# jameshball/kidney-diffusion

Hardware: AMD Instinct MI355X
Metric: denoising-steps/sec (64->256 SR UNet, bs16) (higher is better)
Workload: dtype f32

## Files before the change

kidney-diffusion_amd/csrc/kernels_small.hip:

```cpp
#include "common.h"

namespace kd {

typedef float f32x16 __attribute__((ext_vector_type(16)));
typedef float f32x4 __attribute__((ext_vector_type(4)));

__device__ __forceinline__ float act_s(float v, int act) {
  if (act == ACT_SILU) return v / (1.0f + expf(-v));
  if (act == ACT_GELU) return 0.5f * v * (1.0f + erff(v * 0.70710678118654752440f));
  if (act == ACT_SIGMOID) return 1.0f / (1.0f + expf(-v));
  return v;
}
__device__ __forceinline__ float wave_sum(float v) {
#pragma unroll
  for (int off = 32; off > 0; off >>= 1) v += __shfl_xor(v, off, 64);
  return v;
}

constexpr int SKM_UNROLL = 8;

template <int KW>
__global__ __launch_bounds__(64 * KW) void linear_skinny_mfma_kernel(const float* __restrict__ x, int ldx,
                                                                    const float* __restrict__ w,
                                                                    const float* __restrict__ bias,
                                                                    float* __restrict__ y, int ldy, int M, int K, int N,
                                                                    int in_act, int act) {
  __shared__ float part[KW > 1 ? (KW - 1) * 16 * 64 : 1];
  const int lane = threadIdx.x & 63, i = lane & 31, h = lane >> 5;
  const int kw = threadIdx.x >> 6;
  const int n0 = blockIdx.x * 32, m0 = blockIdx.y * 32;
  const int n = min(n0 + i, N - 1);
  const int m = m0 + i;
  const bool m_ok = m < M;
  const float* wp = w + (int64_t)n * K + 4 * h;
  const float* xp = x + (int64_t)(m_ok ? m : 0) * ldx + 4 * h;
  f32x16 acc;
#pragma unroll
  for (int r = 0; r < 16; ++r) acc[r] = 0.f;
  const f32x4 z = {0.f, 0.f, 0.f, 0.f};
  const int kper = KW > 1 ? ((K + KW * 8 * SKM_UNROLL - 1) / (KW * 8 * SKM_UNROLL)) * (8 * SKM_UNROLL) : K;
  const int k_lo = kw * kper, k_hi = min(K, k_lo + kper);
  for (int k0 = k_lo; k0 < k_hi; k0 += 8 * SKM_UNROLL) {
    f32x4 a[SKM_UNROLL], b[SKM_UNROLL];
#pragma unroll
    for (int u = 0; u < SKM_UNROLL; ++u) {
      int k = k0 + 8 * u + 4 * h;
      bool ok = k < k_hi;
      a[u] = ok ? *(const f32x4*)(wp + k0 + 8 * u) : z;
      b[u] = (ok && m_ok) ? *(const f32x4*)(xp + k0 + 8 * u) : z;
    }
#pragma unroll
    for (int u = 0; u < SKM_UNROLL; ++u) {
      if (in_act != ACT_NONE) {
#pragma unroll
        for (int e = 0; e < 4; ++e) b[u][e] = act_s(b[u][e], in_act);
      }
#pragma unroll
      for (int s = 0; s < 4; ++s) acc = __builtin_amdgcn_mfma_f32_32x32x2f32(a[u][s], b[u][s], acc, 0, 0, 0);
    }
  }
  if (KW > 1) {
    if (kw > 0) {
#pragma unroll
      for (int r = 0; r < 16; ++r) part[((kw - 1) * 16 + r) * 64 + lane] = acc[r];
    }
    __syncthreads();
    if (kw > 0) return;
#pragma unroll
    for (int q = 0; q < KW - 1; ++q)
#pragma unroll
      for (int r = 0; r < 16; ++r) acc[r] += part[(q * 16 + r) * 64 + lane];
  }
  if (!m_ok) return;
  float* yr = y + (int64_t)m * ldy;
  const bool vec = (ldy & 3) == 0 && (((uintptr_t)y) & 15) == 0;
#pragma unroll
  for (int g = 0; g < 4; ++g) {
    const int nb = n0 + 8 * g + 4 * h;
    float v[4];
#pragma unroll
    for (int e = 0; e < 4; ++e) {
      int nn = nb + e;
      v[e] = act_s(acc[4 * g + e] + ((bias && nn < N) ? bias[nn] : 0.f), act);
    }
    if (vec && nb + 3 < N) {
      f32x4 o = {v[0], v[1], v[2], v[3]};
      *(f32x4*)(yr + nb) = o;
    } else {
#pragma unroll
      for (int e = 0; e < 4; ++e)
        if (nb + e < N) yr[nb + e] = v[e];
    }
  }
}

int launch_linear_skinny(const float* x, int ldx, const float* w, const float* bias, float* y, int ldy, int M,
                         int K, int N, int in_act, int act, hipStream_t s) {
  KD_REQUIRE(M > 0 && N > 0 && K > 0, "skinny linear: empty");
  const bool mfma_ok = (K & 3) == 0 && (ldx & 3) == 0 && (((uintptr_t)x) & 15) == 0 && (((uintptr_t)w) & 15) == 0;
  if (!mfma_ok) return launch_linear_skinny_valu(x, ldx, w, bias, y, ldy, M, K, N, in_act, act, s);
  if (M == 1 && K <= 16384) return launch_linear_gemv(x, w, bias, y, K, N, in_act, act, s);
  dim3 grid((N + 31) / 32, (M + 31) / 32);
  if (K >= 512)
    hipLaunchKernelGGL(linear_skinny_mfma_kernel<4>, grid, dim3(256), 0, s, x, ldx, w, bias, y, ldy, M, K, N, in_act, act);
  else
    hipLaunchKernelGGL(linear_skinny_mfma_kernel<1>, grid, dim3(64), 0, s, x, ldx, w, bias, y, ldy, M, K, N, in_act, act);
  KD_HIP_CHECK(hipGetLastError());
  return 0;
}

constexpr int GCA_ROWS = 256;
static inline int gca_rows(int HW, int B) {
  int r = GCA_ROWS;
  while ((HW + r - 1) / r > 1024) r *= 2;
  while (r > 32 && (int64_t)((HW + r - 1) / r) * B < 1024 && (HW + r / 2 - 1) / (r / 2) <= 1024) r /= 2;
  return r;
}
constexpr int GCA_MAXT = 8;
constexpr int GCA_U = 4;

template <int T, int RPW>
__global__ __launch_bounds__(256) void gca_partial_kernel(const float* __restrict__ x, const float* __restrict__ wk,
                                                          const float* __restrict__ bk, float* __restrict__ part,
                                                          int HW, int C, int rows) {
  extern __shared__ float sm[];
  const int b = blockIdx.y, chunk = blockIdx.x, nchunks = gridDim.x;
  const int lane = threadIdx.x & 63, wave = threadIdx.x >> 6;
  constexpr int LPR = 64 / RPW;
  const int sub = RPW == 2 ? (lane >> 5) : 0;
  const int li = RPW == 2 ? (lane & 31) : lane;
  const int C4 = C >> 2;
  const int p0 = chunk * rows, p1 = min(HW, p0 + rows);
  f32x4 wv[T], acc[T];
  const f32x4 z = {0.f, 0.f, 0.f, 0.f};
#pragma unroll
  for (int t = 0; t < T; ++t) {
    int c4 = li + LPR * t;
    wv[t] = c4 < C4 ? *(const f32x4*)(wk + c4 * 4) : z;
    acc[t] = z;
  }
  const float bias = bk[0];
  float mrun = -INFINITY, lrun = 0.f;
  const int stride = 4 * RPW;
  for (int pb = p0 + wave * RPW + sub; pb < p1; pb += stride * GCA_U) {
    f32x4 xv[GCA_U][T];
#pragma unroll
    for (int u = 0; u < GCA_U; ++u) {
      const int p = pb + u * stride;
      const float* xr = x + ((int64_t)b * HW + (p < p1 ? p : p0)) * C;
#pragma unroll
      for (int t = 0; t < T; ++t) {
        int c4 = li + LPR * t;
        xv[u][t] = c4 < C4 ? *(const f32x4*)(xr + c4 * 4) : z;
      }
    }
#pragma unroll
    for (int u = 0; u < GCA_U; ++u) {
      float d = 0.f;
#pragma unroll
      for (int t = 0; t < T; ++t)
        d += (xv[u][t][0] * wv[t][0] + xv[u][t][1] * wv[t][1]) + (xv[u][t][2] * wv[t][2] + xv[u][t][3] * wv[t][3]);
#pragma unroll
      for (int off = LPR / 2; off > 0; off >>= 1) d += __shfl_xor(d, off, 64);
      if (pb + u * stride < p1) {
        const float logit = d + bias;
        const float mnew = fmaxf(mrun, logit);
        const float corr = expf(mrun - mnew), pw = expf(logit - mnew);
        lrun = lrun * corr + pw;
#pragma unroll
        for (int t = 0; t < T; ++t) acc[t] = acc[t] * corr + xv[u][t] * pw;
        mrun = mnew;
      }
    }
  }
  if (RPW == 2) {
    const float mo = __shfl_xor(mrun, 32, 64), lo = __shfl_xor(lrun, 32, 64);
    const float mn = fmaxf(mrun, mo);
    const float e1 = mrun == -INFINITY ? 0.f : expf(mrun - mn), e2 = mo == -INFINITY ? 0.f : expf(mo - mn);
#pragma unroll
    for (int t = 0; t < T; ++t) {
      f32x4 ao;
#pragma unroll
      for (int e = 0; e < 4; ++e) ao[e] = __shfl_xor(acc[t][e], 32, 64);
      acc[t] = acc[t] * e1 + ao * e2;
    }
    lrun = lrun * e1 + lo * e2;
    mrun = mn;
  }
  float* sacc = sm;
  float* sml = sm + 4 * C;
  if (lane == 0) {
    sml[wave * 2] = mrun;
    sml[wave * 2 + 1] = lrun;
  }
  if (sub == 0) {
#pragma unroll
    for (int t = 0; t < T; ++t) {
      int c4 = li + LPR * t;
      if (c4 < C4) *(f32x4*)(sacc + wave * C + c4 * 4) = acc[t];
    }
  }
  __syncthreads();
  float mb = fmaxf(fmaxf(sml[0], sml[2]), fmaxf(sml[4], sml[6]));
  float sc[4], lb = 0.f;
#pragma unroll
  for (int wv_ = 0; wv_ < 4; ++wv_) {
    sc[wv_] = sml[wv_ * 2] == -INFINITY ? 0.f : expf(sml[wv_ * 2] - mb);
    lb += sml[wv_ * 2 + 1] * sc[wv_];
  }
  float* out = part + ((int64_t)b * nchunks + chunk) * (C + 2);
  for (int c = threadIdx.x; c < C; c += 256)
    out[2 + c] = (sacc[c] * sc[0] + sacc[C + c] * sc[1]) + (sacc[2 * C + c] * sc[2] + sacc[3 * C + c] * sc[3]);
  if (threadIdx.x == 0) {
    out[0] = mb;
    out[1] = lb;
  }
}

__global__ __launch_bounds__(256) void gca_combine_kernel(const float* __restrict__ part, float* __restrict__ pooled,
                                                          int nchunks, int C) {
  __shared__ float se[1024];
  __shared__ float red[8];
  __shared__ float sacc[16][16];
  const int b = blockIdx.x, lane = threadIdx.x & 63, wave = threadIdx.x >> 6;
  const int cl = threadIdx.x & 15, sub = threadIdx.x >> 4;
  const int c = blockIdx.y * 16 + cl;
  const float* pb = part + (int64_t)b * nchunks * (C + 2);
  float m = -INFINITY;
  for (int i = threadIdx.x; i < nchunks; i += 256) m = fmaxf(m, pb[(int64_t)i * (C + 2)]);
#pragma unroll
  for (int off = 32; off > 0; off >>= 1) m = fmaxf(m, __shfl_xor(m, off, 64));
  if (lane == 0) red[wave] = m;
  __syncthreads();
  const float mg = fmaxf(fmaxf(red[0], red[1]), fmaxf(red[2], red[3]));
  float l = 0.f;
  for (int i = threadIdx.x; i < nchunks; i += 256) {
    float e = expf(pb[(int64_t)i * (C + 2)] - mg);
    se[i] = e;
    l += pb[(int64_t)i * (C + 2) + 1] * e;
  }
  l = wave_sum(l);
  if (lane == 0) red[4 + wave] = l;
  __syncthreads();
  const float inv = 1.0f / ((red[4] + red[5]) + (red[6] + red[7]));
  float s = 0.f;
  if (c < C)
    for (int i = sub; i < nchunks; i += 16) s += pb[(int64_t)i * (C + 2) + 2 + c] * se[i];
  sacc[sub][cl] = s;
  __syncthreads();
  if (sub == 0 && c < C) {
    float t = 0.f;
#pragma unroll
    for (int k = 0; k < 16; ++k) t += sacc[k][cl];
    pooled[(int64_t)b * C + c] = t * inv;
  }
}

constexpr int GCAG_MAXC = 512;
__global__ __launch_bounds__(256) void gca_gate_kernel(const float* __restrict__ part, int nchunks, int C,
                                                       const float* __restrict__ w0, const float* __restrict__ b0, int hid,
                                                       const float* __restrict__ w2, const float* __restrict__ b2,
                                                       float* __restrict__ gate) {
  __shared__ float se[1024];
  __shared__ float red[8];
  __shared__ __attribute__((aligned(16))) float pooled[GCAG_MAXC];
  __shared__ __attribute__((aligned(16))) float hidden[GCAG_MAXC / 2];
  const int b = blockIdx.x, lane = threadIdx.x & 63, wave = threadIdx.x >> 6;
  const float* pb = part + (int64_t)b * nchunks * (C + 2);
  float m = -INFINITY;
  for (int i = threadIdx.x; i < nchunks; i += 256) m = fmaxf(m, pb[(int64_t)i * (C + 2)]);
#pragma unroll
  for (int off = 32; off > 0; off >>= 1) m = fmaxf(m, __shfl_xor(m, off, 64));
  if (lane == 0) red[wave] = m;
  __syncthreads();
  const float mg = fmaxf(fmaxf(red[0], red[1]), fmaxf(red[2], red[3]));
  float l = 0.f;
  for (int i = threadIdx.x; i < nchunks; i += 256) {
    const float e = expf(pb[(int64_t)i * (C + 2)] - mg);
    se[i] = e;
    l += pb[(int64_t)i * (C + 2) + 1] * e;
  }
  l = wave_sum(l);
  if (lane == 0) red[4 + wave] = l;
  __syncthreads();
  const float inv = 1.0f / ((red[4] + red[5]) + (red[6] + red[7]));
  for (int c = threadIdx.x; c < C; c += 256) {
    float s0 = 0.f, s1 = 0.f, s2 = 0.f, s3 = 0.f;
    int i = 0;
    for (; i + 3 < nchunks; i += 4) {
      s0 = fmaf(pb[(int64_t)i * (C + 2) + 2 + c], se[i], s0);
      s1 = fmaf(pb[(int64_t)(i + 1) * (C + 2) + 2 + c], se[i + 1], s1);
      s2 = fmaf(pb[(int64_t)(i + 2) * (C + 2) + 2 + c], se[i + 2], s2);
      s3 = fmaf(pb[(int64_t)(i + 3) * (C + 2) + 2 + c], se[i + 3], s3);
    }
    for (; i < nchunks; ++i) s0 = fmaf(pb[(int64_t)i * (C + 2) + 2 + c], se[i], s0);
    pooled[c] = ((s0 + s1) + (s2 + s3)) * inv;
  }
  __syncthreads();
  typedef float f32x4g __attribute__((ext_vector_type(4)));
  for (int h = threadIdx.x; h < hid; h += 256) {
    const f32x4g* wr = (const f32x4g*)(w0 + (int64_t)h * C);
    float a0 = 0.f, a1 = 0.f, a2 = 0.f, a3 = 0.f;
    for (int c4 = 0; c4 < C / 4; ++c4) {
      const f32x4g wv = wr[c4], pv = *(const f32x4g*)(pooled + 4 * c4);
      a0 = fmaf(wv[0], pv[0], a0);
      a1 = fmaf(wv[1], pv[1], a1);
      a2 = fmaf(wv[2], pv[2], a2);
      a3 = fmaf(wv[3], pv[3], a3);
    }
    const float v = ((a0 + a1) + (a2 + a3)) + b0[h];
    hidden[h] = v / (1.0f + expf(-v));
  }
  __syncthreads();
  for (int n = threadIdx.x; n < C; n += 256) {
    const float* wr = w2 + (int64_t)n * hid;
    float a0 = 0.f, a1 = 0.f;
    int h = 0;
    if ((hid & 3) == 0) {
      float a2 = 0.f, a3 = 0.f;
      for (; h < hid; h += 4) {
        const f32x4g wv = *(const f32x4g*)(wr + h), hv = *(const f32x4g*)(hidden + h);
        a0 = fmaf(wv[0], hv[0], a0);
        a1 = fmaf(wv[1], hv[1], a1);
        a2 = fmaf(wv[2], hv[2], a2);
        a3 = fmaf(wv[3], hv[3], a3);
      }
      a0 += a2;
      a1 += a3;
    } else {
      for (; h < hid; ++h) a0 = fmaf(wr[h], hidden[h], a0);
    }
    const float v = (a0 + a1) + b2[n];
    gate[(int64_t)b * C + n] = 1.0f / (1.0f + expf(-v));
  }
}

bool gca_gate_fused_ok(int C, int hid) {
  return C % 4 == 0 && C <= GCAG_MAXC && hid <= GCAG_MAXC / 2 && hid > 0;
}

static int launch_gca_partial(const float* x, const float* wk, const float* bk, float* scratch, int B, int HW, int C, int rows,
                              int chunks, hipStream_t s) {
  size_t smem = (size_t)(4 * C + 8) * sizeof(float);
  const int C4 = C / 4;
  dim3 grid(chunks, B), blk(256);
  if (C4 == 32) hipLaunchKernelGGL((gca_partial_kernel<1, 2>), grid, blk, smem, s, x, wk, bk, scratch, HW, C, rows);
  else if (C4 <= 64) hipLaunchKernelGGL((gca_partial_kernel<1, 1>), grid, blk, smem, s, x, wk, bk, scratch, HW, C, rows);
  else if (C4 <= 128) hipLaunchKernelGGL((gca_partial_kernel<2, 1>), grid, blk, smem, s, x, wk, bk, scratch, HW, C, rows);
  else if (C4 <= 256) hipLaunchKernelGGL((gca_partial_kernel<4, 1>), grid, blk, smem, s, x, wk, bk, scratch, HW, C, rows);
  else hipLaunchKernelGGL((gca_partial_kernel<8, 1>), grid, blk, smem, s, x, wk, bk, scratch, HW, C, rows);
  KD_HIP_CHECK(hipGetLastError());
  return 0;
}

int launch_gca_gate(const float* x, const float* wk, const float* bk, float* scratch, const float* w0, const float* b0, int hid,
                    const float* w2, const float* b2, float* gate, int B, int HW, int C, hipStream_t s) {
  KD_REQUIRE(gca_gate_fused_ok(C, hid), "fused GlobalContext gate needs C % 4 == 0, C <= 512, hidden <= 256");
  KD_REQUIRE((((uintptr_t)w0 | (uintptr_t)w2) & 15) == 0, "fused GlobalContext gate: 16-byte aligned weights");
  const int rows = gca_rows(HW, B), chunks = (HW + rows - 1) / rows;
  if (launch_gca_partial(x, wk, bk, scratch, B, HW, C, rows, chunks, s)) return 1;
  hipLaunchKernelGGL(gca_gate_kernel, dim3(B), dim3(256), 0, s, scratch, chunks, C, w0, b0, hid, w2, b2, gate);
  KD_HIP_CHECK(hipGetLastError());
  return 0;
}

size_t gca_scratch_floats(int B, int HW, int C) {
  int rows = gca_rows(HW, B), chunks = (HW + rows - 1) / rows;
  return (size_t)B * chunks * (C + 2);
}

int launch_gca_pool(const float* x, const float* wk, const float* bk, float* , float* pooled,
                    float* scratch, int B, int HW, int C, hipStream_t s) {
  KD_REQUIRE(C % 4 == 0 && C <= 64 * 4 * GCA_MAXT, "gca needs C % 4 == 0 and C <= 2048");
  const int rows = gca_rows(HW, B), chunks = (HW + rows - 1) / rows;
  if (launch_gca_partial(x, wk, bk, scratch, B, HW, C, rows, chunks, s)) return 1;
  hipLaunchKernelGGL(gca_combine_kernel, dim3(B, (C + 15) / 16), dim3(256), 0, s, scratch, pooled, chunks, C);
  KD_HIP_CHECK(hipGetLastError());
  return 0;
}

}
```

Baseline: 40.57.

## Widen GlobalContext gate kernel to 1024 threads with split-K pooling and FC

The fused GlobalContext gate kernel now runs 1024 threads per block instead of 256. The pooled reduction over chunks is split across several thread groups per channel, and both small FC layers split each row's dot product across up to four threads, with partial sums reduced in shared memory. The kernel is launched with only B blocks, so the aim is to raise parallelism in this latency-bound tail. In exchange it adds extra barriers and shared memory, and the reduction order changes slightly.

```diff
diff --git a/kidney-diffusion_amd/csrc/kernels_small.hip b/kidney-diffusion_amd/csrc/kernels_small.hip
--- a/kidney-diffusion_amd/csrc/kernels_small.hip
+++ b/kidney-diffusion_amd/csrc/kernels_small.hip
@@ -257,80 +257,119 @@
 }
 
 constexpr int GCAG_MAXC = 512;
-__global__ __launch_bounds__(256) void gca_gate_kernel(const float* __restrict__ part, int nchunks, int C,
-                                                       const float* __restrict__ w0, const float* __restrict__ b0, int hid,
-                                                       const float* __restrict__ w2, const float* __restrict__ b2,
-                                                       float* __restrict__ gate) {
+constexpr int GCAG_T = 1024;
+typedef float f32x4g __attribute__((ext_vector_type(4)));
+__device__ inline int gcag_row_split(int rows, int len) {
+  int p = 4;
+  while (p > 1 && (rows * p > GCAG_T || (len & (4 * p - 1)) != 0)) p >>= 1;
+  return p;
+}
+__device__ inline float gcag_dot(const float* __restrict__ w, const float* v, int n) {
+  float a0 = 0.f, a1 = 0.f, a2 = 0.f, a3 = 0.f;
+  for (int k = 0; k < n; k += 4) {
+    const f32x4g wv = *(const f32x4g*)(w + k), pv = *(const f32x4g*)(v + k);
+    a0 = fmaf(wv[0], pv[0], a0);
+    a1 = fmaf(wv[1], pv[1], a1);
+    a2 = fmaf(wv[2], pv[2], a2);
+    a3 = fmaf(wv[3], pv[3], a3);
+  }
+  return (a0 + a1) + (a2 + a3);
+}
+__device__ inline void gcag_fc(const float* __restrict__ w, const float* v, int rows, int len, float* part, float* fc) {
+  const int P = gcag_row_split(rows, len);
+  if (P > 1) {
+    const int r = threadIdx.x / P, q = threadIdx.x - r * P, n = len / P;
+    if (r < rows) part[threadIdx.x] = gcag_dot(w + (int64_t)r * len + q * n, v + q * n, n);
+    __syncthreads();
+    if ((int)threadIdx.x < rows) {
+      float t = part[threadIdx.x * P];
+      for (int k = 1; k < P; ++k) t += part[threadIdx.x * P + k];
+      fc[threadIdx.x] = t;
+    }
+  } else {
+    for (int r = threadIdx.x; r < rows; r += GCAG_T) {
+      const float* wr = w + (int64_t)r * len;
+      if ((len & 3) == 0) {
+        fc[r] = gcag_dot(wr, v, len);
+      } else {
+        float a = 0.f;
+        for (int k = 0; k < len; ++k) a = fmaf(wr[k], v[k], a);
+        fc[r] = a;
+      }
+    }
+  }
+}
+
+__global__ __launch_bounds__(GCAG_T) void gca_gate_kernel(const float* __restrict__ part, int nchunks, int C,
+                                                          const float* __restrict__ w0, const float* __restrict__ b0, int hid,
+                                                          const float* __restrict__ w2, const float* __restrict__ b2,
+                                                          float* __restrict__ gate) {
+  constexpr int NT = GCAG_T, NW = NT / 64;
   __shared__ float se[1024];
-  __shared__ float red[8];
+  __shared__ float red[2 * NW];
+  __shared__ float spart[NT];
   __shared__ __attribute__((aligned(16))) float pooled[GCAG_MAXC];
   __shared__ __attribute__((aligned(16))) float hidden[GCAG_MAXC / 2];
-  const int b = blockIdx.x, lane = threadIdx.x & 63, wave = threadIdx.x >> 6;
+  __shared__ float fc[GCAG_MAXC];
+  const int tid = threadIdx.x, b = blockIdx.x, lane = tid & 63, wave = tid >> 6;
   const float* pb = part + (int64_t)b * nchunks * (C + 2);
   float m = -INFINITY;
-  for (int i = threadIdx.x; i < nchunks; i += 256) m = fmaxf(m, pb[(int64_t)i * (C + 2)]);
+  for (int i = tid; i < nchunks; i += NT) m = fmaxf(m, pb[(int64_t)i * (C + 2)]);
 #pragma unroll
   for (int off = 32; off > 0; off >>= 1) m = fmaxf(m, __shfl_xor(m, off, 64));
   if (lane == 0) red[wave] = m;
   __syncthreads();
-  const float mg = fmaxf(fmaxf(red[0], red[1]), fmaxf(red[2], red[3]));
+  float mg = red[0];
+#pragma unroll
+  for (int w = 1; w < NW; ++w) mg = fmaxf(mg, red[w]);
   float l = 0.f;
-  for (int i = threadIdx.x; i < nchunks; i += 256) {
+  for (int i = tid; i < nchunks; i += NT) {
     const float e = expf(pb[(int64_t)i * (C + 2)] - mg);
     se[i] = e;
     l += pb[(int64_t)i * (C + 2) + 1] * e;
   }
   l = wave_sum(l);
-  if (lane == 0) red[4 + wave] = l;
-  __syncthreads();
-  const float inv = 1.0f / ((red[4] + red[5]) + (red[6] + red[7]));
-  for (int c = threadIdx.x; c < C; c += 256) {
+  if (lane == 0) red[NW + wave] = l;
+  __syncthreads();
+  float lsum = red[NW];
+#pragma unroll
+  for (int w = 1; w < NW; ++w) lsum += red[NW + w];
+  const float inv = 1.0f / lsum;
+  const int S = C < NT ? NT / C : 1, per = (nchunks + S - 1) / S;
+  for (int t = tid; t < S * C; t += NT) {
+    const int sub = S > 1 ? t / C : 0, c = t - sub * C;
+    const int i1 = min(nchunks, (sub + 1) * per);
     float s0 = 0.f, s1 = 0.f, s2 = 0.f, s3 = 0.f;
-    int i = 0;
-    for (; i + 3 < nchunks; i += 4) {
+    int i = sub * per;
+    for (; i + 3 < i1; i += 4) {
       s0 = fmaf(pb[(int64_t)i * (C + 2) + 2 + c], se[i], s0);
       s1 = fmaf(pb[(int64_t)(i + 1) * (C + 2) + 2 + c], se[i + 1], s1);
       s2 = fmaf(pb[(int64_t)(i + 2) * (C + 2) + 2 + c], se[i + 2], s2);
       s3 = fmaf(pb[(int64_t)(i + 3) * (C + 2) + 2 + c], se[i + 3], s3);
     }
-    for (; i < nchunks; ++i) s0 = fmaf(pb[(int64_t)i * (C + 2) + 2 + c], se[i], s0);
-    pooled[c] = ((s0 + s1) + (s2 + s3)) * inv;
-  }
-  __syncthreads();
-  typedef float f32x4g __attribute__((ext_vector_type(4)));
-  for (int h = threadIdx.x; h < hid; h += 256) {
-    const f32x4g* wr = (const f32x4g*)(w0 + (int64_t)h * C);
-    float a0 = 0.f, a1 = 0.f, a2 = 0.f, a3 = 0.f;
-    for (int c4 = 0; c4 < C / 4; ++c4) {
-      const f32x4g wv = wr[c4], pv = *(const f32x4g*)(pooled + 4 * c4);
-      a0 = fmaf(wv[0], pv[0], a0);
-      a1 = fmaf(wv[1], pv[1], a1);
-      a2 = fmaf(wv[2], pv[2], a2);
-      a3 = fmaf(wv[3], pv[3], a3);
-    }
-    const float v = ((a0 + a1) + (a2 + a3)) + b0[h];
+    for (; i < i1; ++i) s0 = fmaf(pb[(int64_t)i * (C + 2) + 2 + c], se[i], s0);
+    const float sum = (s0 + s1) + (s2 + s3);
+    if (S > 1) spart[t] = sum;
+    else pooled[c] = sum * inv;
+  }
+  if (S > 1) {
+    __syncthreads();
+    if (tid < C) {
+      float t = spart[tid];
+      for (int k = 1; k < S; ++k) t += spart[k * C + tid];
+      pooled[tid] = t * inv;
+    }
+  }
+  __syncthreads();
+  gcag_fc(w0, pooled, hid, C, spart, fc);
+  for (int h = tid; h < hid; h += NT) {
+    const float v = fc[h] + b0[h];
     hidden[h] = v / (1.0f + expf(-v));
   }
   __syncthreads();
-  for (int n = threadIdx.x; n < C; n += 256) {
-    const float* wr = w2 + (int64_t)n * hid;
-    float a0 = 0.f, a1 = 0.f;
-    int h = 0;
-    if ((hid & 3) == 0) {
-      float a2 = 0.f, a3 = 0.f;
-      for (; h < hid; h += 4) {
-        const f32x4g wv = *(const f32x4g*)(wr + h), hv = *(const f32x4g*)(hidden + h);
-        a0 = fmaf(wv[0], hv[0], a0);
-        a1 = fmaf(wv[1], hv[1], a1);
-        a2 = fmaf(wv[2], hv[2], a2);
-        a3 = fmaf(wv[3], hv[3], a3);
-      }
-      a0 += a2;
-      a1 += a3;
-    } else {
-      for (; h < hid; ++h) a0 = fmaf(wr[h], hidden[h], a0);
-    }
-    const float v = (a0 + a1) + b2[n];
+  gcag_fc(w2, hidden, C, hid, spart, fc);
+  for (int n = tid; n < C; n += NT) {
+    const float v = fc[n] + b2[n];
     gate[(int64_t)b * C + n] = 1.0f / (1.0f + expf(-v));
   }
 }
@@ -359,7 +398,7 @@
   KD_REQUIRE((((uintptr_t)w0 | (uintptr_t)w2) & 15) == 0, "fused GlobalContext gate: 16-byte aligned weights");
   const int rows = gca_rows(HW, B), chunks = (HW + rows - 1) / rows;
   if (launch_gca_partial(x, wk, bk, scratch, B, HW, C, rows, chunks, s)) return 1;
-  hipLaunchKernelGGL(gca_gate_kernel, dim3(B), dim3(256), 0, s, scratch, chunks, C, w0, b0, hid, w2, b2, gate);
+  hipLaunchKernelGGL(gca_gate_kernel, dim3(B), dim3(GCAG_T), 0, s, scratch, chunks, C, w0, b0, hid, w2, b2, gate);
   KD_HIP_CHECK(hipGetLastError());
   return 0;
 }
```

After: 40.76 (median of 6 runs). No clear change (+0.5%).
